# zovoilis-lab/Flye

Measured on AMD Instinct MI355X. Metric: Gbp reads overlapped/sec, higher is better.
Workload: dtype u64

## Files before the change

### flye_amd/csrc/fg_api.hip

```cpp
#include "fg_ctx.h"
#include <chrono>
#include <cmath>

#include <algorithm>
#include <new>

#include <mutex>
#include <atomic>

static std::mutex g_poolMutex;
static std::vector<BatchOwner*> g_pool;

BatchOwner* BatchOwner::acquire()
{
	std::lock_guard<std::mutex> lock(g_poolMutex);
	if (g_pool.empty()) return new BatchOwner;
	BatchOwner* b = g_pool.back();
	g_pool.pop_back();
	return b;
}

void BatchOwner::release(BatchOwner* b)
{
	if (!b) return;
// ... 70 lines not shown
	fg_ctx* c = new (std::nothrow) fg_ctx;
	if (!c) return FG_ERR_NOMEM;
	c->device = device;
	c->k = kmer_size;
	if (hipStreamCreateWithFlags(&c->stream, hipStreamNonBlocking) != hipSuccess ||
		hipStreamCreateWithFlags(&c->stream2, hipStreamNonBlocking) != hipSuccess ||
		hipStreamCreateWithFlags(&c->stream3, hipStreamNonBlocking) != hipSuccess ||
		hipEventCreateWithFlags(&c->evJoin3, hipEventDisableTiming) != hipSuccess ||
		hipEventCreateWithFlags(&c->evOff, hipEventDisableTiming) != hipSuccess ||
		hipEventCreateWithFlags(&c->evFork, hipEventDisableTiming) != hipSuccess ||
		hipEventCreateWithFlags(&c->evJoin, hipEventDisableTiming) != hipSuccess)
	{
		delete c;
		return FG_ERR_NO_DEVICE;
	}
	for (auto& e : c->evPiece)
		if (hipEventCreateWithFlags(&e, hipEventDisableTiming) != hipSuccess) { delete c; return FG_ERR_NO_DEVICE; }
	c->timer.stream = c->stream;
	*out = c;
	return FG_OK;
}

void fg_destroy(fg_ctx* ctx)
{
	if (!ctx) return;
	(void)hipSetDevice(ctx->device);
	(void)hipStreamSynchronize(ctx->stream);
	delete ctx;
}

int fg_container_info(const fg_ctx* c, uint32_t* first_id, uint32_t* n_fwd, uint32_t* query_first_id, uint32_t* query_n_fwd)
{
// ... 1218 lines not shown
```

### flye_amd/csrc/fg_ctx.h

```cpp
#pragma once

#include <hip/hip_runtime.h>
#include <cstdint>
#include <cstdio>
#include <cstdlib>
#include <new>
#include <cstring>
#include <string>
#include <vector>
#include <map>
#include <memory>
#include <condition_variable>
#include <functional>
#include <mutex>
#include <thread>
#include <atomic>
#include <algorithm>

#include "../../include/flye_gpu.h"

typedef uint64_t u64;
typedef uint32_t u32;
typedef int32_t i32;

// ... 217 lines not shown
	~ShimPool()
	{
		{ std::lock_guard<std::mutex> g(mu); stop = true; }
		cvGo.notify_all();
		for (auto& t : threads) if (t.joinable()) t.join();
	}
};

struct fg_ctx {
	int device = 0;
	int k = 17;
	hipStream_t stream = nullptr;
	hipStream_t stream2 = nullptr, stream3 = nullptr;
	hipEvent_t evFork = nullptr, evJoin = nullptr, evJoin3 = nullptr;
#define FG_D2H_MAX_PIECES 16
	hipEvent_t evOff = nullptr, evPiece[FG_D2H_MAX_PIECES] = {};
	unsigned long long pieceEnd[FG_D2H_MAX_PIECES] = {};
	int nPieces = 0;
	std::string lastError;
	KernelTimer timer;

	u32 nReads = 0;
	u32 firstId = 0;
	u64 totalWords = 0, totalBases = 0, totalKmers = 0;
	i32 maxLen = 0;
	std::vector<i32> hLen;
	std::vector<u64> hKmerOff;
	DevBuf<u64> dWords;
	DevBuf<u64> dWordOff;
	DevBuf<i32> dLen;
	DevBuf<u64> dKmerOff;

	bool hasQ = false;
// ... 83 lines not shown
	DevBuf<u64> dTrimRowCnt, dTrimRowOff, dTrimScan, dTrimKeys, dTrimIvl, dTrimSeg, dTrimAcc, dTrimAccOff;
	DevBuf<unsigned long long> dTrimPairCnt;
	DevBuf<u32> dTrimVals, dTrimAccCnt, dTrimKept;
	DevBuf<char> dTrimRaw, dTrimOut;
	DevBuf<u32> dRcNodes, dRcVals, dRcU32;
	DevBuf<char> dRcTab, dRcAln;
	DevBuf<u64> dRcOff, dRcKeys, dRcOut;
	DevBuf<i32> dRcOutScore;
	DevBuf<char> dCovRecs, dCovSort;
	DevBuf<u64> dCovIv, dCovKeys, dCovOff;
	DevBuf<i32> dCovI32, dCovVec;
	DevBuf<char> dPolBytes, dPolCand, dPolItems, dPolTasks, dPolRes;
	DevBuf<u64> dPolOff, dPolEdOff;
	DevBuf<long long> dPolScore, dPolCells, dPolEdits;
	DevBuf<char> dBub[36];
	PinnedBuf<char> hPrim;
	PinnedBuf<u64> hOff;
	PinnedBuf<u64> hScalar;
	ShimPool shimPool;

	~fg_ctx()
	{
		if (evFork) (void)hipEventDestroy(evFork);
		if (evJoin) (void)hipEventDestroy(evJoin);
		if (evJoin3) (void)hipEventDestroy(evJoin3);
		if (evOff) (void)hipEventDestroy(evOff);
		for (auto e : evPiece) if (e) (void)hipEventDestroy(e);
		if (stream2) (void)hipStreamDestroy(stream2);
		if (stream3) (void)hipStreamDestroy(stream3);
		if (stream) (void)hipStreamDestroy(stream);
	}
};

#if defined(__HIPCC__)

__device__ __forceinline__ i32 fg_uni(i32 v) { return __builtin_amdgcn_readfirstlane(v); }
__device__ __forceinline__ u32 fg_uni(u32 v) { return (u32)__builtin_amdgcn_readfirstlane((int)v); }
__device__ __forceinline__ u64 fg_uni(u64 v)
{
	return ((u64)(u32)__builtin_amdgcn_readfirstlane((int)(u32)(v >> 32)) << 32) |
		   (u32)__builtin_amdgcn_readfirstlane((int)(u32)v);
}
// ... 169 lines not shown
	void reserveMatches(size_t nPairs)
	{
		if (nPairs <= matchCap) return;
		free(matches);
		matchCap = nPairs + nPairs / 8 + 16;
		matches = (int32_t*)malloc(matchCap * 8);
		if (!matches) { matchCap = 0; throw std::bad_alloc(); }
	}
	void reserveRecs(size_t n)
	{
		if (n <= recCap) return;
		free(recs);
		recCap = n + n / 8 + 16;
		recs = (fg_overlap_rec*)malloc(recCap * sizeof(fg_overlap_rec));
		if (!recs) { recCap = 0; throw std::bad_alloc(); }
	}
	~BatchOwner() { free(recs); free(matches); }
	static BatchOwner* acquire();
	static void release(BatchOwner* b);
};

struct PrimRec {
	u32 query;
	u32 extId;
	i32 curBegin, curEnd, extBegin, extEnd, extLen, score, chainLength, filtered;
	i32 editDistance, hpcLenCur, hpcLenExt;
};

void fgBuildIndexSolid(fg_ctx* c, i32 minFreq, float selectRate, i32 tandemFreq, float repeatRate,
					   float sampleRateInit, fg_index_stats* st);
// ... 78 lines not shown
```

### flye_amd/csrc/fg_overlap.hip

```cpp
#include "fg_ctx.h"
#include "fg_wavesort.h"
#include "fg_devprim.h"
#include "fg_taskchain.h"
#include <atomic>

#include <algorithm>
#include <cmath>
#include <chrono>
#include <functional>
#include <thread>
#include <type_traits>

#define WG 256
#define FLAG_SELF (1ULL << 63)
#define FLAG_FLIP (1ULL << 62)
#define OFF_MASK ((1ULL << 38) - 1)

namespace {

__device__ __forceinline__ u32 block_exscan(u32 v, u32* sh , u32* total)
{
	const int lane = threadIdx.x & 63, w = threadIdx.x >> 6;
	u32 inc = v;
	for (int o = 1; o < 64; o <<= 1)
// ... 1385 lines not shown
	  if (fgprim::radixSortPairs(s, k0, v0, k1, v1, nHits, 0, onePass ? gBits + storedBits : storedBits, c->dPartScratch.p))
		  { std::swap(k0, k1); std::swap(v0, v1); } }
	if (!onePass)
	{
		{ ScopedK t(c->timer, "k_recv_keys");
		  hipLaunchKernelGGL(k_recv_gkey, (unsigned)((nHits + WG - 1) / WG), WG, 0, s, v0, nHits, c->dHitOff.p, nq, dQKmerOff,
							 recv->hits, c->dRecvIdx.p, k0); }
		ScopedK t(c->timer, "k_recv_sort");
		if (fgprim::radixSortPairs(s, k0, v0, k1, v1, nHits, 0, gBits, c->dPartScratch.p)) { std::swap(k0, k1); std::swap(v0, v1); }
	}
	{ ScopedK t(c->timer, "k_recv_place");
	  hipLaunchKernelGGL(k_recv_place<KT>, (unsigned)((nHits + WG - 1) / WG), WG, 0, s, v0, nHits, recv->hits, c->dRecvIdx.p,
						 c->firstId, curBits, hitKey, hitVal); }
}

static void deviceSub(fg_ctx* c, const fg_detector_params* p, uint8_t forceLocal, u32 sub0, u32 nq, u64 primBase,
					  u64 hitCapHint , ChunkResult* res,
					  const RecvHits* recv = nullptr, u32 callQ0 = 0)
{
	hipStream_t s = c->stream;
	const int k = c->k;
	const u32* dQuery = c->dQuery.p + sub0;
	const u64* dQKmerOff = c->dQKmerOff.p + sub0;
	c->curQuery = dQuery;
	const i32* qLen = c->hasQ ? c->dQLen.p : c->dLen.p;
	c->dHitOff.reserve(nq + 1); c->dFiltOff.reserve(nq + 1);
	c->dGroupCnt.reserve(nq + 1); c->dGroupOff.reserve(nq + 1);
	c->dPrimCnt.reserve(nq + 1); c->dPrimOff.reserve(nq + 1); c->dDpGroups.reserve(nq + 1); c->dDpElems.reserve(nq + 1);
	c->dListCnt.reserve(4);
	{ ScopedK t(c->timer, "k_exscan");
	  hipLaunchKernelGGL(k_exscan, 1, 1024, 0, s, c->dCntA.p + sub0, c->dHitOff.p, nq);
	  hipLaunchKernelGGL(k_exscan, 1, 1024, 0, s, c->dCntB.p + sub0, c->dFiltOff.p, nq); }
	c->hScalar.reserve(8);
	HIP_CHECK(hipMemcpyAsync(c->hScalar.p, c->dHitOff.p + nq, 8, hipMemcpyDeviceToHost, s));
// ... 87 lines not shown
		{ ScopedK t(c->timer, "k_exscan");
		  hipLaunchKernelGGL(k_exscan, 1, 1024, 0, s, c->dMatchSize.p, c->dMatchOff.p, (u32)nPrim); }
		const u64 slots = fetchScalar(c, c->dMatchOff.p + nPrim);
		res->nMatchSlots = slots;
		c->dMatches.reserve(slots + 1);
		{ ScopedK t(c->timer, "k_chain_matches");
		  hipLaunchKernelGGL(k_chain_matches, (unsigned)((nPrim + WG - 1) / WG), WG, 0, s, (const PrimRec*)c->dPrimOut.p, nPrim,
							 c->dPrimNode.p, c->dPrimBase.p, c->dMatchOff.p, c->dCur.p, c->dExt.p, c->dBack.p, k,
							 c->dMatches.p, c->dMatchCnt.p); }
		c->hMatches.reserve(slots + 1); c->hMatchOff.reserve(nPrim + 1); c->hMatchCnt.reserve(nPrim + 1);
		ScopedK t(c->timer, "copy_results_d2h");
		HIP_CHECK(hipMemcpyAsync(c->hMatches.p, c->dMatches.p, slots * 8, hipMemcpyDeviceToHost, s));
		HIP_CHECK(hipMemcpyAsync(c->hMatchOff.p, c->dMatchOff.p, (nPrim + 1) * 8, hipMemcpyDeviceToHost, s));
		HIP_CHECK(hipMemcpyAsync(c->hMatchCnt.p, c->dMatchCnt.p, nPrim * 4, hipMemcpyDeviceToHost, s));
	}
	if ((primBase + nPrim + 1) * sizeof(PrimRec) > c->hPrim.n)
	{
		HIP_CHECK(hipStreamSynchronize(s));
		c->hPrim.reserveKeep((primBase + nPrim + 1) * sizeof(PrimRec), primBase * sizeof(PrimRec));
	}
	c->hOff.reserve(3 * (size_t)(nq + 1) + 1);
	{ ScopedK t(c->timer, "copy_results_d2h");
	  HIP_CHECK(hipMemcpyAsync(c->hOff.p, c->dPrimOff.p, (nq + 1) * 8ULL, hipMemcpyDeviceToHost, s));
	  HIP_CHECK(hipMemcpyAsync(c->hOff.p + (nq + 1), c->dDpGroups.p, nq * 8ULL, hipMemcpyDeviceToHost, s));
	  HIP_CHECK(hipMemcpyAsync(c->hOff.p + 2 * (size_t)(nq + 1), c->dDpElems.p, nq * 8ULL, hipMemcpyDeviceToHost, s));
	  HIP_CHECK(hipMemcpyAsync(c->hOff.p + 3 * (size_t)(nq + 1), c->dSmallElems.p, 8, hipMemcpyDeviceToHost, s));
	  HIP_CHECK(hipEventRecord(c->evOff, s));
	  static const int wantPieces = getenv("FG_D2H_PIECES") ? std::max(1, std::min(FG_D2H_MAX_PIECES, atoi(getenv("FG_D2H_PIECES")))) : 12;
	  const int nPieces = nPrim >= 100000 ? wantPieces : 1;
	  for (int i = 0; i < nPieces; ++i)
	  {
		  const u64 a = nPrim * i / nPieces, b = nPrim * (i + 1) / nPieces;
		  if (b > a)
			  HIP_CHECK(hipMemcpyAsync(c->hPrim.p + (primBase + a) * sizeof(PrimRec), c->dPrimOut.p + a * sizeof(PrimRec),
									   (b - a) * sizeof(PrimRec), hipMemcpyDeviceToHost, s));
		  HIP_CHECK(hipEventRecord(c->evPiece[i], s));
		  c->pieceEnd[i] = primBase + b;
	  }
	  c->nPieces = nPieces; }
	HIP_CHECK(hipEventSynchronize(c->evOff));
	if (keepAln) HIP_CHECK(hipStreamSynchronize(s));
	res->nPrim = nPrim;
	res->dpGroups = 0; res->dpElems = 0;
	res->dpElemsSmall = c->hOff.p[3 * (size_t)(nq + 1)];
	for (u32 i = 0; i < nq; ++i) { res->dpGroups += c->hOff.p[(nq + 1) + i]; res->dpElems += c->hOff.p[2 * (size_t)(nq + 1) + i]; }
}

static void stageBudgets(fg_ctx* c, u64& kmerBudget, u64& hitBudget)
{
	kmerBudget = getenv("FG_KMER_BUDGET") ? strtoull(getenv("FG_KMER_BUDGET"), nullptr, 10) : (1ULL << 30);
	hitBudget = getenv("FG_HIT_BUDGET") ? strtoull(getenv("FG_HIT_BUDGET"), nullptr, 10) : (3ULL << 29);
	if (!getenv("FG_KMER_BUDGET") && !getenv("FG_HIT_BUDGET"))
	{
		size_t freeB = 0, totalB = 0;
// ... 9 lines not shown

static fg_ctx* laneTwo(fg_ctx* c)
{
	if (!c->lane2)
	{
		std::unique_ptr<fg_ctx> l(new fg_ctx);
		l->device = c->device;
		if (hipStreamCreateWithFlags(&l->stream, hipStreamNonBlocking) != hipSuccess ||
			hipStreamCreateWithFlags(&l->stream2, hipStreamNonBlocking) != hipSuccess ||
			hipStreamCreateWithFlags(&l->stream3, hipStreamNonBlocking) != hipSuccess ||
			hipEventCreateWithFlags(&l->evJoin3, hipEventDisableTiming) != hipSuccess ||
			hipEventCreateWithFlags(&l->evOff, hipEventDisableTiming) != hipSuccess ||
			hipEventCreateWithFlags(&l->evFork, hipEventDisableTiming) != hipSuccess ||
			hipEventCreateWithFlags(&l->evJoin, hipEventDisableTiming) != hipSuccess)
			throw FgError{FG_ERR_HIP, "streams of the second lane"};
		for (auto& e : l->evPiece)
			if (hipEventCreateWithFlags(&e, hipEventDisableTiming) != hipSuccess) throw FgError{FG_ERR_HIP, "events of the second lane"};
		l->timer.stream = l->stream;
		c->lane2 = std::move(l);
	}
	fg_ctx* l = c->lane2.get();
	l->k = c->k; l->nReads = c->nReads; l->firstId = c->firstId; l->maxLen = c->maxLen;
	l->totalKmers = c->totalKmers; l->totalBases = c->totalBases;
	l->hasQ = c->hasQ; l->nQReads = c->nQReads; l->qFirstId = c->qFirstId; l->qMaxLen = c->qMaxLen;
	l->indexBuilt = c->indexBuilt; l->sampleRate = c->sampleRate; l->nKeys = c->nKeys; l->nEntries = c->nEntries; l->nRep = c->nRep;
	l->tableSlots = c->tableSlots; l->tableWide = c->tableWide; l->table = c->table;
	l->timer.enabled = c->timer.enabled;
	l->dWords.alias(c->dWords); l->dWordOff.alias(c->dWordOff); l->dLen.alias(c->dLen); l->dKmerOff.alias(c->dKmerOff);
	l->dQWords.alias(c->dQWords); l->dQWordOff.alias(c->dQWordOff); l->dQLen.alias(c->dQLen);
	l->dKeyOff.alias(c->dKeyOff); l->dEntries.alias(c->dEntries); l->dTable.alias(c->dTable); l->dIndexedBits.alias(c->dIndexedBits); l->dMaybeBits.alias(c->dMaybeBits);
	l->dQuery.alias(c->dQuery); l->dQKmerOff.alias(c->dQKmerOff); l->dProbe.alias(c->dProbe);
	l->dCntA.alias(c->dCntA); l->dCntB.alias(c->dCntB);
	return l;
}

struct SubResult {
	u32 qa = 0, qb = 0;
	int lane = 0;
	u64 lanePrimBase = 0;
	ChunkResult cr{};
	std::vector<u64> primOff;
	std::vector<u64> mData, mOff;
};

void fgOverlaps(fg_ctx* c, const fg_detector_params* p, const u32* queryIds, u32 nq, i32 maxOverlaps,
				uint8_t forceLocal, fg_overlap_batch* out, const RecvHits* recv)
{
	hipStream_t s = c->stream;
	const int k = c->k;
	c->timer.reset();
	c->hitCapHint = 0;
	const auto tHost0 = std::chrono::steady_clock::now();
	struct EvPair {
		KernelTimer& t; hipEvent_t a, b;
		explicit EvPair(KernelTimer& t_) : t(t_), a(t_.get()), b(nullptr) { try { b = t_.get(); } catch (...) { t_.pool.push_back(a); throw; } }
		~EvPair() { t.pool.push_back(a); t.pool.push_back(b); }
	} evp(c->timer);
	const hipEvent_t evA = evp.a, evB = evp.b;
	HIP_CHECK(hipEventRecord(evA, s));
// ... 40 lines not shown
	std::vector<std::pair<u32, u32>> chunks;
	{
		u32 qa = 0;
		while (qa < nq)
		{
			u32 qb = qa + 1;
			while (qb < nq && hQKmerOff[qb + 1] - hQKmerOff[qa] <= kmerBudget) ++qb;
			chunks.push_back({qa, qb});
			qa = qb;
		}
	}
	const bool keepAln = p->keep_alignment;
	std::vector<u64> mData, mOff(1, 0);
	std::vector<u64> primOffAll(nq + 1, 0);
	std::vector<const PrimRec*> primPtr(nq, nullptr);
	std::vector<u64> hitsPerQuery;
	u64 nPrim = 0;
	out->seed_hits = 0; out->dp_groups = 0; out->dp_elements = 0; out->dp_elements_small = 0;
	const int nLanes = getenv("FG_LANES") ? std::max(1, std::min(2, atoi(getenv("FG_LANES")))) : 2;
	const u64 laneMinHits = getenv("FG_LANE_MIN_HITS") ? strtoull(getenv("FG_LANE_MIN_HITS"), nullptr, 10) : (48ULL << 20);
	const u32 laneSplit = getenv("FG_LANE_SPLIT") ? (u32)std::max(2, atoi(getenv("FG_LANE_SPLIT"))) : 4u;
	bool laned = false;
	u64 lanePrim[2] = {0, 0};
	std::vector<std::unique_ptr<SubResult>> subs;
	for (const auto& ch : chunks)
	{
		probeChunk(c, hq.data(), hQKmerOff.data(), ch.first, ch.second, hitsPerQuery);
		const u32 cn = ch.second - ch.first;
		if (recv)
		{
			hitsPerQuery.assign(recv->total + ch.first, recv->total + ch.second);
			HIP_CHECK(hipMemcpyAsync(c->dCntA.p, hitsPerQuery.data(), cn * 8ULL, hipMemcpyHostToDevice, s));
			HIP_CHECK(hipStreamSynchronize(s));
		}
		u64 chunkHits = 0;
		for (u32 i = 0; i < cn; ++i) chunkHits += hitsPerQuery[i];
		const bool forcedCut = getenv("FG_LANE_MIN_HITS") && chunkHits >= laneMinHits && cn >= 2 * laneSplit;
		const bool twoLanes = nLanes == 2 && (chunkHits > hitBudget || forcedCut);
		const u64 budget = !twoLanes ? hitBudget
			: (chunkHits > hitBudget ? std::max<u64>(1, hitBudget / 2) : std::max<u64>(1, (chunkHits + laneSplit - 1) / laneSplit));
		std::vector<std::pair<u32, u32>> ranges;
		u64 maxSubHits = 0;
		std::vector<u64> cuts;
		if (twoLanes && getenv("FG_LANE_FRACS") && chunkHits / 2 <= hitBudget)
		{
			u64 accPct = 0;
			for (const char* q = getenv("FG_LANE_FRACS"); *q;)
			{
				accPct += strtoull(q, (char**)&q, 10);
				if (*q == ',') ++q;
				cuts.push_back(chunkHits / 100 * std::min<u64>(accPct, 100));
			}
		}
		size_t cutI = 0;
		u64 before = 0;
		for (u32 sa = 0; sa < cn;)
		{
			u32 sb = sa + 1;
			u64 acc = hitsPerQuery[sa];
			if (!cuts.empty())
			{
				const u64 upTo = cutI + 1 < cuts.size() ? cuts[cutI] : chunkHits;
				while (sb < cn && before + acc + hitsPerQuery[sb] <= upTo) acc += hitsPerQuery[sb++];
				if (cutI + 1 >= cuts.size()) { while (sb < cn) acc += hitsPerQuery[sb++]; }
				++cutI;
			}
			else
				while (sb < cn && acc + hitsPerQuery[sb] <= budget) acc += hitsPerQuery[sb++];
			ranges.push_back({sa, sb});
			maxSubHits = std::max(maxSubHits, acc);
			before += acc;
			sa = sb;
		}
		const size_t sub0Index = subs.size();
		for (auto& r : ranges)
		{
			subs.emplace_back(new SubResult);
			subs.back()->qa = ch.first + r.first; subs.back()->qb = ch.first + r.second;
		}
		fg_ctx* lanes[2] = {c, nullptr};
		const bool useTwo = twoLanes && ranges.size() >= 2;
		if (useTwo) { lanes[1] = laneTwo(c); if (!laned) lanes[1]->timer.reset(); laned = true; }
		std::atomic<size_t> next{0};
		std::exception_ptr laneErr[2];
		auto work = [&](int lane)
		{
			try
			{
				fg_ctx* lc = lanes[lane];
				(void)hipSetDevice(lc->device);
				while (true)
				{
					const size_t i = next.fetch_add(1);
					if (i >= ranges.size()) break;
					SubResult& sr = *subs[sub0Index + i];
					sr.lane = lane;
					sr.lanePrimBase = lanePrim[lane];
					deviceSub(lc, p, forceLocal, ranges[i].first, ranges[i].second - ranges[i].first, lanePrim[lane], maxSubHits, &sr.cr,
							  recv, ch.first);
					const u32 n = ranges[i].second - ranges[i].first;
					sr.primOff.assign(lc->hOff.p, lc->hOff.p + n + 1);
					if (keepAln)
					{
						sr.mOff.assign(1, 0);
						sr.mData.reserve(sr.cr.nMatchSlots);
						for (u64 j = 0; j < sr.cr.nPrim; ++j)
						{
							const u64 slotEnd = lc->hMatchOff.p[j + 1];
							const u32 cnt = lc->hMatchCnt.p[j];
							sr.mData.insert(sr.mData.end(), lc->hMatches.p + slotEnd - cnt, lc->hMatches.p + slotEnd);
							sr.mOff.push_back(sr.mData.size());
						}
					}
					lanePrim[lane] += sr.cr.nPrim;
				}
				if (useTwo) HIP_CHECK(hipStreamSynchronize(lc->stream));
			}
			catch (...) { laneErr[lane] = std::current_exception(); }
		};
		if (useTwo)
		{
			std::thread helper(work, 1);
			work(0);
			helper.join();
		}
		else work(0);
		for (int l = 0; l < 2; ++l) if (laneErr[l]) std::rethrow_exception(laneErr[l]);
	}
	for (auto& srp : subs)
	{
		SubResult& sr = *srp;
		fg_ctx* lc = sr.lane ? c->lane2.get() : c;
		const PrimRec* base = (const PrimRec*)lc->hPrim.p + sr.lanePrimBase;
		for (u32 i = 0; i < sr.qb - sr.qa; ++i)
		{
			primOffAll[sr.qa + i + 1] = nPrim + sr.primOff[i + 1];
			primPtr[sr.qa + i] = base - nPrim;
		}
		if (keepAln)
			for (u64 j = 0; j < sr.cr.nPrim; ++j)
			{
				mData.insert(mData.end(), sr.mData.begin() + sr.mOff[j], sr.mData.begin() + sr.mOff[j + 1]);
				mOff.push_back(mData.size());
			}
		out->seed_hits += sr.cr.nHits; out->dp_groups += sr.cr.dpGroups; out->dp_elements += sr.cr.dpElems;
		out->dp_elements_small += sr.cr.dpElemsSmall;
		nPrim += sr.cr.nPrim;
	}
	HIP_CHECK(hipEventRecord(evB, s));
	const u64* hPrimOff = primOffAll.data();
	const auto tHost1 = std::chrono::steady_clock::now();
	const int dev = c->device;
	const bool pieceWait = !laned && subs.size() <= 1;
	auto waitPrim = [c, dev, pieceWait](u64 endIdx)
	{
		if (!pieceWait) return;
		(void)hipSetDevice(dev);
		for (int i = 0; i < c->nPieces; ++i)
			if (c->pieceEnd[i] >= endIdx || i == c->nPieces - 1)
			{
				const hipError_t e = hipEventSynchronize(c->evPiece[i]);
				if (e != hipSuccess) throw FgError{FG_ERR_HIP, std::string("waiting for the result copy: ") + hipGetErrorString(e)};
				return;
			}
	};

	const float sampleRate = c->sampleRate;
	const float maxDiv = p->max_divergence;
	const bool nucl = p->nucl_alignment;
	const bool partition = p->partition_bad_mappings;
	const u32 TASK_Q = 128;
	const u32 nTasks = (nq + TASK_Q - 1) / TASK_Q;
	const unsigned usableCpus = fg_usable_cpus();
	unsigned nThreads = std::max(1u, std::min(usableCpus, 32u));
	if (getenv("FG_SHIM_THREADS")) nThreads = std::max(1, atoi(getenv("FG_SHIM_THREADS")));
	if (nPrim < 20000) nThreads = 1;
	nThreads = std::min(nThreads, nTasks);
	own->reserveRecs(nPrim);
	if (partition) own->needsTrim.assign(nPrim, 0);
	if (keepAln) { own->reserveMatches(mData.size()); own->matchOff.assign(nPrim + 1, 0); }
	own->stats.resize(statCap);
	enum { SUM_RECS, SUM_STATS, SUM_MATCHES };
	struct Wnd { i32 range; float div; };
	struct Scratch {
		std::vector<float> div; std::vector<uint8_t> keep;
		std::vector<u32> nRec, nStat;
		std::vector<float> stat;
		std::vector<Wnd> wnd;
	};
	std::vector<Scratch> scratch(nThreads);
	FgTaskChain<3> chain(nTasks);
	auto worker = [&](unsigned th)
	{
		Scratch& S = scratch[th];
		auto count = [&](u32 task, uint64_t* mine)
		{
			const u32 q0 = task * TASK_Q, q1 = std::min(nq, q0 + TASK_Q);
			waitPrim(hPrimOff[q1]);
			const u64 j0 = hPrimOff[q0];
			S.div.resize(hPrimOff[q1] - j0); S.keep.resize(hPrimOff[q1] - j0);
			S.nRec.resize(q1 - q0); S.nStat.resize(q1 - q0);
			S.stat.clear();
			float* div = S.div.data() - j0;
			uint8_t* keep = S.keep.data() - j0;
			for (u32 qi = q0; qi < q1; ++qi)
			{
				const i32 curLen = (c->hasQ ? c->hQLen : c->hLen)[hq[qi] >> 1];
				S.wnd.assign(curLen / STAT_WND + 1, Wnd{0, 0.0f});
				size_t detected = 0;
				u32 prevExt = 0xFFFFFFFFu;
				const PrimRec* hPrim = primPtr[qi];
				for (u64 j = hPrimOff[qi]; j < hPrimOff[qi + 1]; ++j)
				{
// ... 15 lines not shown
						d = (float)r.editDistance / std::max((size_t)r.hpcLenExt, (size_t)r.hpcLenCur);
					div[j] = d;
					if (d < maxDiv) { keep[j] = 1; ++detected; }
					else if (partition) { keep[j] = 2; ++detected; }
					else keep[j] = 0;
					if (keep[j] && keepAln) mine[SUM_MATCHES] += mOff[j + 1] - mOff[j];
					const size_t w = r.curBegin / STAT_WND;
					if (r.curEnd - r.curBegin > S.wnd[w].range) { S.wnd[w].range = r.curEnd - r.curBegin; S.wnd[w].div = d; }
				}
				u32 ns = 0;
				for (auto& w : S.wnd) if (w.range > 0) { S.stat.push_back(w.div); ++ns; }
				S.nRec[qi - q0] = (u32)detected; S.nStat[qi - q0] = ns;
				mine[SUM_RECS] += detected; mine[SUM_STATS] += ns;
			}
		};
		auto write = [&](u32 task, const uint64_t* base)
		{
			const u32 q0 = task * TASK_Q, q1 = std::min(nq, q0 + TASK_Q);
			const u64 j0 = hPrimOff[q0];
			const float* div = S.div.data() - j0;
			const uint8_t* keep = S.keep.data() - j0;
			if (!S.stat.empty()) memcpy(own->stats.data() + base[SUM_STATS], S.stat.data(), S.stat.size() * sizeof(float));
			u64 recAt = base[SUM_RECS], statAt = base[SUM_STATS], mo = base[SUM_MATCHES];
			for (u32 qi = q0; qi < q1; ++qi)
			{
				const i32 curLen = (c->hasQ ? c->hQLen : c->hLen)[hq[qi] >> 1];
				fg_overlap_rec* dst = own->recs + recAt;
				recAt += S.nRec[qi - q0]; statAt += S.nStat[qi - q0];
				own->queryOff[qi + 1] = recAt;
				own->statOff[qi + 1] = statAt;
// ... 15 lines not shown
					o.cur_begin = r.curBegin; o.cur_end = r.curEnd; o.cur_len = curLen;
					o.ext_begin = r.extBegin; o.ext_end = r.extEnd; o.ext_len = r.extLen;
					o.score = r.score; o.seq_divergence = div[j];
					o.chain_length = r.chainLength; o.filtered_positions = r.filtered;
					o.edit_distance = r.editDistance; o.hpc_len_cur = r.hpcLenCur; o.hpc_len_ext = r.hpcLenExt;
					static_assert(sizeof(fg_overlap_rec) % 4 == 0, "record of 32-bit fields");
					const int* src32 = (const int*)&o;
					int* dst32 = (int*)dst;
#pragma unroll
					for (unsigned w4 = 0; w4 < sizeof(fg_overlap_rec) / 4; ++w4) __builtin_nontemporal_store(src32[w4], dst32 + w4);
					++dst;
				}
			}
			__builtin_ia32_sfence();
		};
		chain.work(count, write);
	};
	if (!pieceWait) HIP_CHECK(hipStreamSynchronize(s));
	c->shimPool.run(nThreads, worker);
	chain.rethrow();
	HIP_CHECK(hipStreamSynchronize(s));
	own->nRecs = chain.total(SUM_RECS);
	own->stats.resize(chain.total(SUM_STATS));
	if (partition) own->needsTrim.resize(own->nRecs);
	if (keepAln) { own->matchOff.resize(own->nRecs + 1); own->matchOff[own->nRecs] = chain.total(SUM_MATCHES); }
	out->n_recs = own->nRecs;
	out->query_off = own->queryOff.data();
	out->recs = own->recs;
	out->n_div_stats = own->stats.size();
	out->div_stats_off = own->statOff.data();
	out->div_stats = own->stats.data();
	if (partition) out->needs_trim = own->needsTrim.data();
	if (keepAln)
	{
// ... 101 lines not shown
```

### flye_amd/csrc/fg_taskchain.h

```cpp
#pragma once
#include <atomic>
#include <cstdint>
#include <exception>
#include <memory>
#include <mutex>
#include <thread>

template <int N>
struct FgTaskChain {
	struct alignas(64) Slot {
		std::atomic<uint32_t> ready{0};
		uint64_t sum[N];
	};
	std::unique_ptr<Slot[]> slots;
	uint32_t nTasks = 0;
	std::atomic<uint32_t> next{0};
	std::atomic<bool> failed{false};
	std::mutex errMu;
	std::exception_ptr err;

	explicit FgTaskChain(uint32_t n) : slots(n ? new Slot[n] : nullptr), nTasks(n) {}

	void fail(std::exception_ptr e)
	{
		std::lock_guard<std::mutex> g(errMu);
		if (!err) err = e;
		failed.store(true, std::memory_order_release);
	}

	template <class Count, class Write>
	void work(Count&& count, Write&& write)
	{
		while (true)
		{
			const uint32_t t = next.fetch_add(1, std::memory_order_relaxed);
			if (t >= nTasks) return;
			uint64_t mine[N] = {}, base[N] = {};
			bool counted = false;
			if (!failed.load(std::memory_order_acquire))
			{
				try { count(t, mine); counted = true; }
				catch (...) { for (int i = 0; i < N; ++i) mine[i] = 0; fail(std::current_exception()); }
			}
			if (t)
			{
				const Slot& prev = slots[t - 1];
				for (unsigned spins = 0; !prev.ready.load(std::memory_order_acquire); ++spins)
				{
					if (spins < 64) __builtin_ia32_pause();
					else std::this_thread::yield();
				}
				for (int i = 0; i < N; ++i) base[i] = prev.sum[i];
			}
			Slot& me = slots[t];
			for (int i = 0; i < N; ++i) me.sum[i] = base[i] + mine[i];
			me.ready.store(1, std::memory_order_release);
			if (counted && !failed.load(std::memory_order_acquire))
			{
				try { write(t, base); }
				catch (...) { fail(std::current_exception()); }
			}
		}
	}

	uint64_t total(int i) const { return nTasks ? slots[nTasks - 1].sum[i] : 0; }
	void rethrow() { if (err) std::rethrow_exception(err); }
};
```

Baseline: 4.508.

## Stream host record assembly concurrently with later GPU sub-ranges

Host-side overlap record assembly (the shim worker pool) now starts after the first chunk and runs alongside the remaining GPU sub-range launches. It waits on a publication board and on per-sub D2H piece events instead of running only after every sub-range has finished. Each sub-range gets its own pinned result slab and event set, so the shared growing pinned buffer and its synchronous reallocation are gone. Output records go into an arena that grows on demand from an estimate, which can cost extra reallocation and copying. The added threads, locks and ordering logic bring some risk of contention or stalls.

```diff
diff --git a/flye_amd/csrc/fg_api.hip b/flye_amd/csrc/fg_api.hip
--- a/flye_amd/csrc/fg_api.hip
+++ b/flye_amd/csrc/fg_api.hip
@@ -108,8 +108,6 @@
 		delete c;
 		return FG_ERR_NO_DEVICE;
 	}
-	for (auto& e : c->evPiece)
-		if (hipEventCreateWithFlags(&e, hipEventDisableTiming) != hipSuccess) { delete c; return FG_ERR_NO_DEVICE; }
 	c->timer.stream = c->stream;
 	*out = c;
 	return FG_OK;
diff --git a/flye_amd/csrc/fg_ctx.h b/flye_amd/csrc/fg_ctx.h
--- a/flye_amd/csrc/fg_ctx.h
+++ b/flye_amd/csrc/fg_ctx.h
@@ -255,9 +255,9 @@
 	hipStream_t stream2 = nullptr, stream3 = nullptr;
 	hipEvent_t evFork = nullptr, evJoin = nullptr, evJoin3 = nullptr;
 #define FG_D2H_MAX_PIECES 16
-	hipEvent_t evOff = nullptr, evPiece[FG_D2H_MAX_PIECES] = {};
-	unsigned long long pieceEnd[FG_D2H_MAX_PIECES] = {};
-	int nPieces = 0;
+	hipEvent_t evOff = nullptr;
+	std::vector<hipEvent_t> evSub;
+	u32 subsThisCall = 0, slabGrows = 0;
 	std::string lastError;
 	KernelTimer timer;
 
@@ -371,7 +371,7 @@
 	DevBuf<u64> dPolOff, dPolEdOff;
 	DevBuf<long long> dPolScore, dPolCells, dPolEdits;
 	DevBuf<char> dBub[36];
-	PinnedBuf<char> hPrim;
+	std::vector<std::unique_ptr<PinnedBuf<char>>> hPrimSlabs;
 	PinnedBuf<u64> hOff;
 	PinnedBuf<u64> hScalar;
 	ShimPool shimPool;
@@ -382,7 +382,7 @@
 		if (evJoin) (void)hipEventDestroy(evJoin);
 		if (evJoin3) (void)hipEventDestroy(evJoin3);
 		if (evOff) (void)hipEventDestroy(evOff);
-		for (auto e : evPiece) if (e) (void)hipEventDestroy(e);
+		for (auto e : evSub) if (e) (void)hipEventDestroy(e);
 		if (stream2) (void)hipStreamDestroy(stream2);
 		if (stream3) (void)hipStreamDestroy(stream3);
 		if (stream) (void)hipStreamDestroy(stream);
@@ -582,6 +582,15 @@
 		recCap = n + n / 8 + 16;
 		recs = (fg_overlap_rec*)malloc(recCap * sizeof(fg_overlap_rec));
 		if (!recs) { recCap = 0; throw std::bad_alloc(); }
+	}
+	void growRecs(size_t newCap, size_t keep)
+	{
+		if (newCap <= recCap) return;
+		fg_overlap_rec* q = (fg_overlap_rec*)malloc(newCap * sizeof(fg_overlap_rec));
+		if (!q) throw std::bad_alloc();
+		if (keep) memcpy(q, recs, keep * sizeof(fg_overlap_rec));
+		free(recs);
+		recs = q; recCap = newCap;
 	}
 	~BatchOwner() { free(recs); free(matches); }
 	static BatchOwner* acquire();
diff --git a/flye_amd/csrc/fg_overlap.hip b/flye_amd/csrc/fg_overlap.hip
--- a/flye_amd/csrc/fg_overlap.hip
+++ b/flye_amd/csrc/fg_overlap.hip
@@ -2,6 +2,7 @@
 #include "fg_wavesort.h"
 #include "fg_devprim.h"
 #include "fg_taskchain.h"
+#include "fg_subtail.h"
 #include <atomic>
 
 #include <algorithm>
@@ -1423,10 +1424,24 @@
 						 c->firstId, curBits, hitKey, hitVal); }
 }
 
-static void deviceSub(fg_ctx* c, const fg_detector_params* p, uint8_t forceLocal, u32 sub0, u32 nq, u64 primBase,
-					  u64 hitCapHint , ChunkResult* res,
+
+struct SubResult {
+	u32 qa = 0, qb = 0;
+	const PrimRec* prims = nullptr;
+	hipEvent_t evPiece[FG_D2H_MAX_PIECES] = {};
+	u64 pieceEnd[FG_D2H_MAX_PIECES] = {};
+	int nPieces = 0;
+	u64 primBase = 0;
+	ChunkResult cr{};
+	std::vector<u64> primOff;
+	std::vector<u64> mData, mOff;
+};
+
+static void deviceSub(fg_ctx* c, const fg_detector_params* p, uint8_t forceLocal, u32 sub0, u32 nq, SubResult* sr,
+					  u64 hitCapHint ,
 					  const RecvHits* recv = nullptr, u32 callQ0 = 0)
 {
+	ChunkResult* res = &sr->cr;
 	hipStream_t s = c->stream;
 	const int k = c->k;
 	const u32* dQuery = c->dQuery.p + sub0;
@@ -1544,11 +1559,18 @@
 		HIP_CHECK(hipMemcpyAsync(c->hMatchOff.p, c->dMatchOff.p, (nPrim + 1) * 8, hipMemcpyDeviceToHost, s));
 		HIP_CHECK(hipMemcpyAsync(c->hMatchCnt.p, c->dMatchCnt.p, nPrim * 4, hipMemcpyDeviceToHost, s));
 	}
-	if ((primBase + nPrim + 1) * sizeof(PrimRec) > c->hPrim.n)
-	{
-		HIP_CHECK(hipStreamSynchronize(s));
-		c->hPrim.reserveKeep((primBase + nPrim + 1) * sizeof(PrimRec), primBase * sizeof(PrimRec));
-	}
+	const u32 slot = c->subsThisCall++;
+	while (c->hPrimSlabs.size() <= slot) c->hPrimSlabs.emplace_back(new PinnedBuf<char>);
+	PinnedBuf<char>& slab = *c->hPrimSlabs[slot];
+	if ((nPrim + 1) * sizeof(PrimRec) > slab.n) { slab.reserve((nPrim + 1) * sizeof(PrimRec)); ++c->slabGrows; }
+	while (c->evSub.size() < (size_t)(slot + 1) * FG_D2H_MAX_PIECES)
+	{
+		hipEvent_t e = nullptr;
+		HIP_CHECK(hipEventCreateWithFlags(&e, hipEventDisableTiming));
+		c->evSub.push_back(e);
+	}
+	for (int i = 0; i < FG_D2H_MAX_PIECES; ++i) sr->evPiece[i] = c->evSub[(size_t)slot * FG_D2H_MAX_PIECES + i];
+	sr->prims = (const PrimRec*)slab.p;
 	c->hOff.reserve(3 * (size_t)(nq + 1) + 1);
 	{ ScopedK t(c->timer, "copy_results_d2h");
 	  HIP_CHECK(hipMemcpyAsync(c->hOff.p, c->dPrimOff.p, (nq + 1) * 8ULL, hipMemcpyDeviceToHost, s));
@@ -1562,12 +1584,12 @@
 	  {
 		  const u64 a = nPrim * i / nPieces, b = nPrim * (i + 1) / nPieces;
 		  if (b > a)
-			  HIP_CHECK(hipMemcpyAsync(c->hPrim.p + (primBase + a) * sizeof(PrimRec), c->dPrimOut.p + a * sizeof(PrimRec),
+			  HIP_CHECK(hipMemcpyAsync(slab.p + a * sizeof(PrimRec), c->dPrimOut.p + a * sizeof(PrimRec),
 									   (b - a) * sizeof(PrimRec), hipMemcpyDeviceToHost, s));
-		  HIP_CHECK(hipEventRecord(c->evPiece[i], s));
-		  c->pieceEnd[i] = primBase + b;
+		  HIP_CHECK(hipEventRecord(sr->evPiece[i], s));
+		  sr->pieceEnd[i] = b;
 	  }
-	  c->nPieces = nPieces; }
+	  sr->nPieces = nPieces; }
 	HIP_CHECK(hipEventSynchronize(c->evOff));
 	if (keepAln) HIP_CHECK(hipStreamSynchronize(s));
 	res->nPrim = nPrim;
@@ -1607,8 +1629,6 @@
 			hipEventCreateWithFlags(&l->evFork, hipEventDisableTiming) != hipSuccess ||
 			hipEventCreateWithFlags(&l->evJoin, hipEventDisableTiming) != hipSuccess)
 			throw FgError{FG_ERR_HIP, "streams of the second lane"};
-		for (auto& e : l->evPiece)
-			if (hipEventCreateWithFlags(&e, hipEventDisableTiming) != hipSuccess) throw FgError{FG_ERR_HIP, "events of the second lane"};
 		l->timer.stream = l->stream;
 		c->lane2 = std::move(l);
 	}
@@ -1627,15 +1647,6 @@
 	return l;
 }
 
-struct SubResult {
-	u32 qa = 0, qb = 0;
-	int lane = 0;
-	u64 lanePrimBase = 0;
-	ChunkResult cr{};
-	std::vector<u64> primOff;
-	std::vector<u64> mData, mOff;
-};
-
 void fgOverlaps(fg_ctx* c, const fg_detector_params* p, const u32* queryIds, u32 nq, i32 maxOverlaps,
 				uint8_t forceLocal, fg_overlap_batch* out, const RecvHits* recv)
 {
@@ -1706,6 +1717,7 @@
 	std::vector<u64> mData, mOff(1, 0);
 	std::vector<u64> primOffAll(nq + 1, 0);
 	std::vector<const PrimRec*> primPtr(nq, nullptr);
+	std::vector<const SubResult*> subOf(nq, nullptr);
 	std::vector<u64> hitsPerQuery;
 	u64 nPrim = 0;
 	out->seed_hits = 0; out->dp_groups = 0; out->dp_elements = 0; out->dp_elements_small = 0;
@@ -1713,164 +1725,58 @@
 	const u64 laneMinHits = getenv("FG_LANE_MIN_HITS") ? strtoull(getenv("FG_LANE_MIN_HITS"), nullptr, 10) : (48ULL << 20);
 	const u32 laneSplit = getenv("FG_LANE_SPLIT") ? (u32)std::max(2, atoi(getenv("FG_LANE_SPLIT"))) : 4u;
 	bool laned = false;
-	u64 lanePrim[2] = {0, 0};
+	c->subsThisCall = 0; c->slabGrows = 0;
 	std::vector<std::unique_ptr<SubResult>> subs;
-	for (const auto& ch : chunks)
-	{
-		probeChunk(c, hq.data(), hQKmerOff.data(), ch.first, ch.second, hitsPerQuery);
-		const u32 cn = ch.second - ch.first;
-		if (recv)
-		{
-			hitsPerQuery.assign(recv->total + ch.first, recv->total + ch.second);
-			HIP_CHECK(hipMemcpyAsync(c->dCntA.p, hitsPerQuery.data(), cn * 8ULL, hipMemcpyHostToDevice, s));
-			HIP_CHECK(hipStreamSynchronize(s));
-		}
-		u64 chunkHits = 0;
-		for (u32 i = 0; i < cn; ++i) chunkHits += hitsPerQuery[i];
-		const bool forcedCut = getenv("FG_LANE_MIN_HITS") && chunkHits >= laneMinHits && cn >= 2 * laneSplit;
-		const bool twoLanes = nLanes == 2 && (chunkHits > hitBudget || forcedCut);
-		const u64 budget = !twoLanes ? hitBudget
-			: (chunkHits > hitBudget ? std::max<u64>(1, hitBudget / 2) : std::max<u64>(1, (chunkHits + laneSplit - 1) / laneSplit));
-		std::vector<std::pair<u32, u32>> ranges;
-		u64 maxSubHits = 0;
-		std::vector<u64> cuts;
-		if (twoLanes && getenv("FG_LANE_FRACS") && chunkHits / 2 <= hitBudget)
-		{
-			u64 accPct = 0;
-			for (const char* q = getenv("FG_LANE_FRACS"); *q;)
-			{
-				accPct += strtoull(q, (char**)&q, 10);
-				if (*q == ',') ++q;
-				cuts.push_back(chunkHits / 100 * std::min<u64>(accPct, 100));
-			}
-		}
-		size_t cutI = 0;
-		u64 before = 0;
-		for (u32 sa = 0; sa < cn;)
-		{
-			u32 sb = sa + 1;
-			u64 acc = hitsPerQuery[sa];
-			if (!cuts.empty())
-			{
-				const u64 upTo = cutI + 1 < cuts.size() ? cuts[cutI] : chunkHits;
-				while (sb < cn && before + acc + hitsPerQuery[sb] <= upTo) acc += hitsPerQuery[sb++];
-				if (cutI + 1 >= cuts.size()) { while (sb < cn) acc += hitsPerQuery[sb++]; }
-				++cutI;
-			}
-			else
-				while (sb < cn && acc + hitsPerQuery[sb] <= budget) acc += hitsPerQuery[sb++];
-			ranges.push_back({sa, sb});
-			maxSubHits = std::max(maxSubHits, acc);
-			before += acc;
-			sa = sb;
-		}
-		const size_t sub0Index = subs.size();
-		for (auto& r : ranges)
-		{
-			subs.emplace_back(new SubResult);
-			subs.back()->qa = ch.first + r.first; subs.back()->qb = ch.first + r.second;
-		}
-		fg_ctx* lanes[2] = {c, nullptr};
-		const bool useTwo = twoLanes && ranges.size() >= 2;
-		if (useTwo) { lanes[1] = laneTwo(c); if (!laned) lanes[1]->timer.reset(); laned = true; }
-		std::atomic<size_t> next{0};
-		std::exception_ptr laneErr[2];
-		auto work = [&](int lane)
-		{
-			try
-			{
-				fg_ctx* lc = lanes[lane];
-				(void)hipSetDevice(lc->device);
-				while (true)
-				{
-					const size_t i = next.fetch_add(1);
-					if (i >= ranges.size()) break;
-					SubResult& sr = *subs[sub0Index + i];
-					sr.lane = lane;
-					sr.lanePrimBase = lanePrim[lane];
-					deviceSub(lc, p, forceLocal, ranges[i].first, ranges[i].second - ranges[i].first, lanePrim[lane], maxSubHits, &sr.cr,
-							  recv, ch.first);
-					const u32 n = ranges[i].second - ranges[i].first;
-					sr.primOff.assign(lc->hOff.p, lc->hOff.p + n + 1);
-					if (keepAln)
-					{
-						sr.mOff.assign(1, 0);
-						sr.mData.reserve(sr.cr.nMatchSlots);
-						for (u64 j = 0; j < sr.cr.nPrim; ++j)
-						{
-							const u64 slotEnd = lc->hMatchOff.p[j + 1];
-							const u32 cnt = lc->hMatchCnt.p[j];
-							sr.mData.insert(sr.mData.end(), lc->hMatches.p + slotEnd - cnt, lc->hMatches.p + slotEnd);
-							sr.mOff.push_back(sr.mData.size());
-						}
-					}
-					lanePrim[lane] += sr.cr.nPrim;
-				}
-				if (useTwo) HIP_CHECK(hipStreamSynchronize(lc->stream));
-			}
-			catch (...) { laneErr[lane] = std::current_exception(); }
-		};
-		if (useTwo)
-		{
-			std::thread helper(work, 1);
-			work(0);
-			helper.join();
-		}
-		else work(0);
-		for (int l = 0; l < 2; ++l) if (laneErr[l]) std::rethrow_exception(laneErr[l]);
-	}
-	for (auto& srp : subs)
-	{
-		SubResult& sr = *srp;
-		fg_ctx* lc = sr.lane ? c->lane2.get() : c;
-		const PrimRec* base = (const PrimRec*)lc->hPrim.p + sr.lanePrimBase;
+	FgSubBoard board;
+	FgArenaGate arena;
+	std::atomic<u64> probedHits{0}, probedKmers{0};
+	u64 pubHits = 0;
+	auto publish = [&](size_t j)
+	{
+		SubResult& sr = *subs[j];
+		sr.primBase = nPrim;
 		for (u32 i = 0; i < sr.qb - sr.qa; ++i)
 		{
 			primOffAll[sr.qa + i + 1] = nPrim + sr.primOff[i + 1];
-			primPtr[sr.qa + i] = base - nPrim;
+			primPtr[sr.qa + i] = sr.prims - nPrim;
+			subOf[sr.qa + i] = &sr;
 		}
 		if (keepAln)
-			for (u64 j = 0; j < sr.cr.nPrim; ++j)
-			{
-				mData.insert(mData.end(), sr.mData.begin() + sr.mOff[j], sr.mData.begin() + sr.mOff[j + 1]);
+			for (u64 m = 0; m < sr.cr.nPrim; ++m)
+			{
+				mData.insert(mData.end(), sr.mData.begin() + sr.mOff[m], sr.mData.begin() + sr.mOff[m + 1]);
 				mOff.push_back(mData.size());
 			}
 		out->seed_hits += sr.cr.nHits; out->dp_groups += sr.cr.dpGroups; out->dp_elements += sr.cr.dpElems;
 		out->dp_elements_small += sr.cr.dpElemsSmall;
 		nPrim += sr.cr.nPrim;
-	}
-	HIP_CHECK(hipEventRecord(evB, s));
-	const u64* hPrimOff = primOffAll.data();
-	const auto tHost1 = std::chrono::steady_clock::now();
+		pubHits += sr.cr.nHits;
+		const u64 pk = probedKmers.load(), ph = probedHits.load();
+		const double callHits = pk ? (double)ph * (double)hQKmerOff[nq] / (double)pk : 0.0;
+		const u64 est = pubHits ? (u64)((double)nPrim * std::max(1.0, callHits / (double)pubHits) * 1.1) : nPrim;
+		if (est > arena.want.load(std::memory_order_relaxed)) arena.want.store(est, std::memory_order_relaxed);
+	};
+
 	const int dev = c->device;
-	const bool pieceWait = !laned && subs.size() <= 1;
-	auto waitPrim = [c, dev, pieceWait](u64 endIdx)
-	{
-		if (!pieceWait) return;
+	auto waitSub = [dev](const SubResult& sr, u64 endIdx)
+	{
 		(void)hipSetDevice(dev);
-		for (int i = 0; i < c->nPieces; ++i)
-			if (c->pieceEnd[i] >= endIdx || i == c->nPieces - 1)
-			{
-				const hipError_t e = hipEventSynchronize(c->evPiece[i]);
+		for (int i = 0; i < sr.nPieces; ++i)
+			if (sr.pieceEnd[i] >= endIdx || i == sr.nPieces - 1)
+			{
+				const hipError_t e = hipEventSynchronize(sr.evPiece[i]);
 				if (e != hipSuccess) throw FgError{FG_ERR_HIP, std::string("waiting for the result copy: ") + hipGetErrorString(e)};
 				return;
 			}
 	};
-
+	const u64* hPrimOff = primOffAll.data();
 	const float sampleRate = c->sampleRate;
 	const float maxDiv = p->max_divergence;
 	const bool nucl = p->nucl_alignment;
 	const bool partition = p->partition_bad_mappings;
 	const u32 TASK_Q = 128;
 	const u32 nTasks = (nq + TASK_Q - 1) / TASK_Q;
-	const unsigned usableCpus = fg_usable_cpus();
-	unsigned nThreads = std::max(1u, std::min(usableCpus, 32u));
-	if (getenv("FG_SHIM_THREADS")) nThreads = std::max(1, atoi(getenv("FG_SHIM_THREADS")));
-	if (nPrim < 20000) nThreads = 1;
-	nThreads = std::min(nThreads, nTasks);
-	own->reserveRecs(nPrim);
-	if (partition) own->needsTrim.assign(nPrim, 0);
-	if (keepAln) { own->reserveMatches(mData.size()); own->matchOff.assign(nPrim + 1, 0); }
+	unsigned nThreads = 1;
 	own->stats.resize(statCap);
 	enum { SUM_RECS, SUM_STATS, SUM_MATCHES };
 	struct Wnd { i32 range; float div; };
@@ -1880,7 +1786,7 @@
 		std::vector<float> stat;
 		std::vector<Wnd> wnd;
 	};
-	std::vector<Scratch> scratch(nThreads);
+	std::vector<Scratch> scratch;
 	FgTaskChain<3> chain(nTasks);
 	auto worker = [&](unsigned th)
 	{
@@ -1888,7 +1794,13 @@
 		auto count = [&](u32 task, uint64_t* mine)
 		{
 			const u32 q0 = task * TASK_Q, q1 = std::min(nq, q0 + TASK_Q);
-			waitPrim(hPrimOff[q1]);
+			if (!board.waitQueries(q1)) throw FgError{FG_ERR_HIP, "a sub-range of the call failed"};
+			for (u32 qi = q0; qi < q1;)
+			{
+				const SubResult& sr = *subOf[qi];
+				waitSub(sr, hPrimOff[std::min(q1, sr.qb)] - sr.primBase);
+				qi = sr.qb;
+			}
 			const u64 j0 = hPrimOff[q0];
 			S.div.resize(hPrimOff[q1] - j0); S.keep.resize(hPrimOff[q1] - j0);
 			S.nRec.resize(q1 - q0); S.nStat.resize(q1 - q0);
@@ -1934,6 +1846,14 @@
 				mine[SUM_RECS] += detected; mine[SUM_STATS] += ns;
 			}
 		};
+		auto place = [&](u32 task, const uint64_t* base, const uint64_t* mine)
+		{
+			arena.place(task, base[SUM_RECS], base[SUM_RECS] + mine[SUM_RECS], chain.finished, [&](u64 newCap, u64 keepRecs)
+			{
+				own->growRecs(newCap, keepRecs);
+				if (partition) own->needsTrim.resize(newCap);
+			});
+		};
 		auto write = [&](u32 task, const uint64_t* base)
 		{
 			const u32 q0 = task * TASK_Q, q1 = std::min(nq, q0 + TASK_Q);
@@ -1979,10 +1899,164 @@
 			}
 			__builtin_ia32_sfence();
 		};
-		chain.work(count, write);
+		chain.work(count, place, write);
 	};
-	if (!pieceWait) HIP_CHECK(hipStreamSynchronize(s));
-	c->shimPool.run(nThreads, worker);
+	auto shimThreads = [&](bool small)
+	{
+		unsigned n = std::max(1u, std::min(fg_usable_cpus(), 32u));
+		if (getenv("FG_SHIM_THREADS")) n = std::max(1, atoi(getenv("FG_SHIM_THREADS")));
+		if (small) n = 1;
+		return std::min(n, nTasks);
+	};
+	struct ShimJoin {
+		FgSubBoard& board; std::thread th;
+		void join() { if (th.joinable()) th.join(); }
+		~ShimJoin() { if (th.joinable()) { board.fail(); th.join(); } }
+	} shim{board, {}};
+	bool streaming = false;
+	for (const auto& ch : chunks)
+	{
+		probeChunk(c, hq.data(), hQKmerOff.data(), ch.first, ch.second, hitsPerQuery);
+		const u32 cn = ch.second - ch.first;
+		if (recv)
+		{
+			hitsPerQuery.assign(recv->total + ch.first, recv->total + ch.second);
+			HIP_CHECK(hipMemcpyAsync(c->dCntA.p, hitsPerQuery.data(), cn * 8ULL, hipMemcpyHostToDevice, s));
+			HIP_CHECK(hipStreamSynchronize(s));
+		}
+		u64 chunkHits = 0;
+		for (u32 i = 0; i < cn; ++i) chunkHits += hitsPerQuery[i];
+		const FgLaneCut cut = fgLaneCut(nLanes, chunkHits, cn, hitBudget, getenv("FG_LANE_MIN_HITS") != nullptr, laneMinHits, laneSplit);
+		const bool twoLanes = cut.twoLanes;
+		const u64 budget = cut.budget;
+		std::vector<std::pair<u32, u32>> ranges;
+		u64 maxSubHits = 0;
+		std::vector<u64> cuts;
+		if (twoLanes && getenv("FG_LANE_FRACS") && chunkHits / 2 <= hitBudget)
+		{
+			u64 accPct = 0;
+			for (const char* q = getenv("FG_LANE_FRACS"); *q;)
+			{
+				accPct += strtoull(q, (char**)&q, 10);
+				if (*q == ',') ++q;
+				cuts.push_back(chunkHits / 100 * std::min<u64>(accPct, 100));
+			}
+		}
+		size_t cutI = 0;
+		u64 before = 0;
+		for (u32 sa = 0; sa < cn;)
+		{
+			u32 sb = sa + 1;
+			u64 acc = hitsPerQuery[sa];
+			if (!cuts.empty())
+			{
+				const u64 upTo = cutI + 1 < cuts.size() ? cuts[cutI] : chunkHits;
+				while (sb < cn && before + acc + hitsPerQuery[sb] <= upTo) acc += hitsPerQuery[sb++];
+				if (cutI + 1 >= cuts.size()) { while (sb < cn) acc += hitsPerQuery[sb++]; }
+				++cutI;
+			}
+			else
+				while (sb < cn && acc + hitsPerQuery[sb] <= budget) acc += hitsPerQuery[sb++];
+			ranges.push_back({sa, sb});
+			maxSubHits = std::max(maxSubHits, acc);
+			before += acc;
+			sa = sb;
+		}
+		const size_t sub0Index = subs.size();
+		for (auto& r : ranges)
+		{
+			subs.emplace_back(new SubResult);
+			subs.back()->qa = ch.first + r.first; subs.back()->qb = ch.first + r.second;
+			board.announce(subs.back()->qa, subs.back()->qb);
+		}
+		probedHits += chunkHits; probedKmers = hQKmerOff[ch.second];
+		if (&ch == &chunks.front() && !keepAln && (chunks.size() > 1 || ranges.size() > 1) &&
+			!(getenv("FG_STREAM_TAIL") && atoi(getenv("FG_STREAM_TAIL")) == 0))
+		{
+			streaming = true;
+			nThreads = shimThreads(false);
+			scratch.resize(nThreads);
+			arena.cap = own->recCap;
+			if (partition) own->needsTrim.resize(own->recCap);
+			shim.th = std::thread([&]
+			{
+				try { c->shimPool.run(nThreads, worker); }
+				catch (...) { chain.fail(std::current_exception()); }
+			});
+		}
+		fg_ctx* lanes[2] = {c, nullptr};
+		const bool useTwo = twoLanes && ranges.size() >= 2;
+		if (useTwo)
+		{
+			lanes[1] = laneTwo(c);
+			if (!laned) { lanes[1]->timer.reset(); lanes[1]->subsThisCall = 0; lanes[1]->slabGrows = 0; }
+			laned = true;
+		}
+		std::atomic<size_t> next{0};
+		std::exception_ptr laneErr[2];
+		auto work = [&](int lane)
+		{
+			try
+			{
+				fg_ctx* lc = lanes[lane];
+				(void)hipSetDevice(lc->device);
+				while (true)
+				{
+					const size_t i = next.fetch_add(1);
+					if (i >= ranges.size()) break;
+					SubResult& sr = *subs[sub0Index + i];
+					const u32 n = ranges[i].second - ranges[i].first;
+					deviceSub(lc, p, forceLocal, ranges[i].first, n, &sr, maxSubHits, recv, ch.first);
+					sr.primOff.assign(lc->hOff.p, lc->hOff.p + n + 1);
+					if (keepAln)
+					{
+						sr.mOff.assign(1, 0);
+						sr.mData.reserve(sr.cr.nMatchSlots);
+						for (u64 j = 0; j < sr.cr.nPrim; ++j)
+						{
+							const u64 slotEnd = lc->hMatchOff.p[j + 1];
+							const u32 cnt = lc->hMatchCnt.p[j];
+							sr.mData.insert(sr.mData.end(), lc->hMatches.p + slotEnd - cnt, lc->hMatches.p + slotEnd);
+							sr.mOff.push_back(sr.mData.size());
+						}
+					}
+					board.done(sub0Index + i, publish);
+				}
+				if (useTwo) HIP_CHECK(hipStreamSynchronize(lc->stream));
+			}
+			catch (...) { laneErr[lane] = std::current_exception(); board.fail(); }
+		};
+		if (useTwo)
+		{
+			std::thread helper(work, 1);
+			work(0);
+			helper.join();
+		}
+		else work(0);
+		for (int l = 0; l < 2; ++l) if (laneErr[l]) std::rethrow_exception(laneErr[l]);
+	}
+	HIP_CHECK(hipEventRecord(evB, s));
+	const auto tHost1 = std::chrono::steady_clock::now();
+	if (streaming) shim.join();
+	else
+	{
+		nThreads = shimThreads(nPrim < 20000);
+		scratch.resize(nThreads);
+		own->reserveRecs(nPrim);
+		arena.cap = arena.reserved = own->recCap;
+		arena.want.store(nPrim);
+		if (partition) own->needsTrim.assign(nPrim, 0);
+		if (keepAln) { own->reserveMatches(mData.size()); own->matchOff.assign(nPrim + 1, 0); }
+		c->shimPool.run(nThreads, worker);
+	}
+	if (getenv("FG_TAIL_LOG"))
+	{
+		std::string prims;
+		for (size_t i = 0; i < subs.size() && i < 16; ++i) prims += (i ? "," : "") + std::to_string(subs[i]->cr.nPrim);
+		fprintf(stderr, "fg_overlaps tail: sub_ranges=%zu lanes=%d streamed=%d slab_grows=%u arena_exceeded=%u arena_grows=%u "
+				"sub_prims=%s\n", subs.size(), laned ? 2 : 1, (int)streaming, c->slabGrows + (laned ? c->lane2->slabGrows : 0u),
+				arena.exceeded, arena.grows, prims.c_str());
+	}
 	chain.rethrow();
 	HIP_CHECK(hipStreamSynchronize(s));
 	own->nRecs = chain.total(SUM_RECS);
diff --git a/flye_amd/csrc/fg_subtail.h b/flye_amd/csrc/fg_subtail.h
--- /dev/null
+++ b/flye_amd/csrc/fg_subtail.h
@@ -0,0 +1,90 @@
+#pragma once
+#include <algorithm>
+#include <atomic>
+#include <condition_variable>
+#include <cstdint>
+#include <mutex>
+#include <thread>
+#include <vector>
+
+struct FgSubBoard {
+	enum State : uint8_t { PENDING, DONE };
+	struct Sub { uint32_t qa, qb; State state; };
+	std::mutex mu;
+	std::condition_variable cv;
+	std::vector<Sub> subs;
+	size_t nextPub = 0;
+	uint32_t publishedQ = 0;
+	bool failed = false;
+
+	size_t announce(uint32_t qa, uint32_t qb)
+	{
+		std::lock_guard<std::mutex> g(mu);
+		subs.push_back(Sub{qa, qb, PENDING});
+		return subs.size() - 1;
+	}
+	template <class Publish>
+	void done(size_t i, Publish&& publish)
+	{
+		std::lock_guard<std::mutex> g(mu);
+		subs[i].state = DONE;
+		bool any = false;
+		while (nextPub < subs.size() && subs[nextPub].state == DONE)
+		{
+			publish(nextPub);
+			publishedQ = subs[nextPub].qb;
+			++nextPub;
+			any = true;
+		}
+		if (any) cv.notify_all();
+	}
+	void fail()
+	{
+		{ std::lock_guard<std::mutex> g(mu); failed = true; }
+		cv.notify_all();
+	}
+	bool waitQueries(uint32_t q1)
+	{
+		std::unique_lock<std::mutex> lk(mu);
+		cv.wait(lk, [&] { return failed || publishedQ >= q1; });
+		return publishedQ >= q1;
+	}
+};
+
+struct FgArenaGate {
+	std::atomic<uint64_t> want{0};
+	uint64_t cap = 0, reserved = 0;
+	uint32_t exceeded = 0, grows = 0;
+
+	template <class Grow>
+	void place(uint32_t task, uint64_t begin, uint64_t end, const std::atomic<uint32_t>& finished, Grow&& grow)
+	{
+		if (end <= reserved) return;
+		if (reserved) ++exceeded;
+		const uint64_t need = std::max(end, want.load(std::memory_order_relaxed));
+		const uint64_t newRes = need + need / 8 + 16;
+		if (newRes > cap)
+		{
+			for (unsigned spins = 0; finished.load(std::memory_order_acquire) < task; ++spins)
+			{
+				if (spins < 64) __builtin_ia32_pause();
+				else std::this_thread::yield();
+			}
+			grow(newRes, begin);
+			cap = newRes;
+			++grows;
+		}
+		reserved = newRes;
+	}
+};
+
+struct FgLaneCut { bool twoLanes; uint64_t budget; };
+inline FgLaneCut fgLaneCut(int nLanes, uint64_t chunkHits, uint32_t nQueries, uint64_t hitBudget, bool forced, uint64_t minHits,
+						   uint32_t split)
+{
+	const bool forcedCut = forced && chunkHits >= minHits && nQueries >= 2 * split;
+	const bool two = nLanes == 2 && (chunkHits > hitBudget || forcedCut);
+	const uint64_t budget = !two ? hitBudget
+		: (chunkHits > hitBudget ? std::max<uint64_t>(1, hitBudget / 2) : std::max<uint64_t>(1, (chunkHits + split - 1) / split));
+	return FgLaneCut{two, budget};
+}
diff --git a/flye_amd/csrc/fg_taskchain.h b/flye_amd/csrc/fg_taskchain.h
--- a/flye_amd/csrc/fg_taskchain.h
+++ b/flye_amd/csrc/fg_taskchain.h
@@ -15,6 +15,7 @@
 	std::unique_ptr<Slot[]> slots;
 	uint32_t nTasks = 0;
 	std::atomic<uint32_t> next{0};
+	std::atomic<uint32_t> finished{0};
 	std::atomic<bool> failed{false};
 	std::mutex errMu;
 	std::exception_ptr err;
@@ -29,7 +30,10 @@
 	}
 
 	template <class Count, class Write>
-	void work(Count&& count, Write&& write)
+	void work(Count&& count, Write&& write) { work(count, [](uint32_t, const uint64_t*, const uint64_t*) {}, write); }
+
+	template <class Count, class Place, class Write>
+	void work(Count&& count, Place&& place, Write&& write)
 	{
 		while (true)
 		{
@@ -52,6 +56,11 @@
 				}
 				for (int i = 0; i < N; ++i) base[i] = prev.sum[i];
 			}
+			if (counted && !failed.load(std::memory_order_acquire))
+			{
+				try { place(t, base, mine); }
+				catch (...) { for (int i = 0; i < N; ++i) mine[i] = 0; counted = false; fail(std::current_exception()); }
+			}
 			Slot& me = slots[t];
 			for (int i = 0; i < N; ++i) me.sum[i] = base[i] + mine[i];
 			me.ready.store(1, std::memory_order_release);
@@ -60,6 +69,7 @@
 				try { write(t, base); }
 				catch (...) { fail(std::current_exception()); }
 			}
+			finished.fetch_add(1, std::memory_order_release);
 		}
 	}
 
```

Result: no change. 4.512, median of 5 (+0.1%).
